# Lucaskabela/UNAST

Hardware: AMD Instinct MI355X
Metric: mel-frames/sec/node (train step, gen+disc) at B=32,T_mel=800; 1/2/4/8-GPU scaling (higher is better)
Workload: dtype bf16x3

## Files before the change

include/unast_hip.h:

```cpp
#ifndef UNAST_HIP_H
#define UNAST_HIP_H
#include <stdint.h>
#ifdef __cplusplus
extern "C" {
#endif

typedef struct ihipStream_t* hipStream_t;

const char* unast_last_error(void);
int unast_version(void);
const char* unast_arch(void);

int unast_gemm(int a_mode, int b_mode, int nsplit,
               const float* A, int lda, const float* B, int ldb, float* C, int ldc,
               int M, int N, int K, int kb_valid,
               int conv_T, int conv_ca, int conv_cb, int conv_shift,
               const float* bias, const float* R, int ldr, const float* G, int ldg, float gate_scale,
               float alpha, int beta, int act,
               float drop_p, unsigned int seed, unsigned int stream_id,
               int splitk, float* splitk_ws, int64_t splitk_ws_floats, float* rowsum_a, int tile_wn, int b_presplit,
               int out_split, double* colstats, hipStream_t stream);

int unast_attn_fwd(int nsplit, const float* Q, int ldq, const float* K, int ldk, const float* V, int ldv, float* O, int ldo,
                   float* LSE, const int* lens_k, int B, int H, int Tq, int Tk, int head_dim, int causal, float scale,
// ... 74 lines not shown
                       hipStream_t stream);

int unast_scalar_combine(const float* a, const float* b, const float* c, float div, float* out, hipStream_t stream);
int unast_masked_mse(const float* gold, const float* pred, const float* mask, int64_t n, double* ws3, float* out, hipStream_t stream);
int unast_speech_loss_fwd(const float* gold, const float* head, int ldh, const float* post, const int* lens, int B, int T, int M,
                          float eos_weight, double* ws, float* loss, hipStream_t stream);
int unast_speech_loss_bwd(const float* gold, const float* head, int ldh, const float* post, const int* lens, int B, int T, int M,
                          float eos_weight, const float* gscale, float* d_head, float* d_post, hipStream_t stream);
int unast_text_loss_fwd(const float* logits, int ldl, const int64_t* gold, int rows, int V, float eos_weight,
                        double* ws, float* loss, hipStream_t stream);
int unast_text_loss_bwd(const float* logits, int ldl, const int64_t* gold, int rows, int V, float eos_weight, const double* ws,
                        const float* gscale, float* dlogits, hipStream_t stream);
int unast_text_head_loss(const float* X, int ldx, const float* W, const float* bias, const int64_t* gold, int rows, int K, int V,
                         float eos_weight, float gscale, float* logits, float* dlogits, int ldl, double* ws, float* loss, hipStream_t stream);
int unast_speech_head_loss(const float* X, int ldx, const float* W, const float* bias, const float* gold, const int* lens, int B, int T, int K, int M,
                           float eos_weight, float gscale, float* head, float* d_head, int ldh, double* ws, hipStream_t stream);
int unast_speech_post_loss(const float* gold, const float* post, const int* lens, int B, int T, int M, float gscale, float* d_post, double* ws,
                           float* loss, hipStream_t stream);
int unast_disc_targets(const int64_t* perm, int n, int B, int flip, float smoothing, float* out, hipStream_t stream);
int unast_randperm(int64_t* out, int n, unsigned int seed, unsigned int stream_id, hipStream_t stream);
int unast_bce_logits(const float* logits, int ldx, const float* targets, int n, const float* gscale, float* loss, float* dlogits,
                     int ldd, hipStream_t stream);

int unast_lstm_fwd(const float* xproj, const float* whh, const float* b_ih, const float* b_hh, const int* lens, float* y, float* gates,
                   float* cs, float* hprev, float* hfinal, int Bd, int T, int ndir, int hidden, int64_t whh_dir_stride,
                   int64_t bias_dir_stride, hipStream_t stream);
int unast_lstm_bwd(const float* dy, const float* dhfinal, const float* whh, const float* gates, const float* cs, const int* lens,
                   float* dgates, int Bd, int T, int ndir, int hidden, int64_t whh_dir_stride, hipStream_t stream);
int unast_leaky_dropout(const float* x, const float* dy, float* out, int rows, int D, float slope, float drop_p, unsigned int seed,
                        unsigned int stream_id, hipStream_t stream);

int unast_conv_fwd(int nsplit, const float* X, int ldx, const float* Wp, float* Y, int ldy, int B, int T, int Cin, int Cout,
                   int taps, int pad_left, const float* bias, int act, const float* R, int ldr, hipStream_t stream);
int unast_maxpool_prev(const float* in, int ld_in, float* out, int ld_out, int B, int T, int C, hipStream_t stream);
int unast_highway_combine(const float* ht, int ld_ht, const float* x, int ld_x, float* out, int ld_out, int rows, int C, hipStream_t stream);
int unast_gru_fwd(const float* xproj, const float* whh, const float* b_hn, float* y, int B, int T, int hidden, hipStream_t stream);

int unast_gru_fwd_train(const float* xproj, const float* whh, const float* b_hn, float* y, float* saved, int B, int T, int hidden,
                        hipStream_t stream);
int unast_gru_bwd(const float* dy, const float* y, const float* saved, const float* whh, float* dx_gates, float* dhn, int B, int T,
                  int hidden, hipStream_t stream);
int unast_maxpool_prev_bwd(const float* dy, int ld_dy, const float* x, int ld_x, float* dx, int ld_dx, int B, int T, int C,
                           int accumulate, int relu_gate, hipStream_t stream);
int unast_relu_bwd(float* dy, int ld_dy, const float* y, int ld_y, int rows, int C, hipStream_t stream);
int unast_highway_combine_bwd(const float* dout, int ld_do, const float* ht, int ld_ht, const float* x, int ld_x, float* dpre, int ld_dp,
                              float* dx, int ld_dx, int rows, int C, hipStream_t stream);
int unast_sum_loss(const float* pred, int ld_pred, const float* mag, int ld_mag, float* dpred, int ld_dpred, int rows, int F, int l2,
                   double* loss, hipStream_t stream);
int unast_split_parts(const float* x, float* hi, float* rest, float* resid, int64_t n, hipStream_t stream);
int unast_conv_dgrad(int nsplit, const float* dY, int lddy, const float* Wp, float* dX, int lddx, int B, int T, int Cin, int Cout,
                     int taps, int pad_left, int beta, hipStream_t stream);
int unast_conv_wgrad(int nsplit, const float* dY, int lddy, const float* X, int ldx, float* dWp, int B, int T, int Cin, int Cout,
                     int taps, int pad_left, float* db, int splitk, float* ws, int64_t ws_floats, hipStream_t stream);

int unast_set_rng_epoch(const unsigned int* counter);

typedef struct {
    const float* A; int lda;
    const float* B; int ldb;
    float* C; int ldc;
    float* rowsum_a;
    int M, N, K;
} unast_wgrad_item;
int unast_wgrad_group(int nsplit, int count, const unast_wgrad_item* items, float* ws, int64_t ws_floats, int target_blocks,
                      hipStream_t stream);
int64_t unast_wgrad_group_ws_floats(int count, const unast_wgrad_item* items, int target_blocks);

int unast_sumsq(const float* g, int64_t n, double* out, hipStream_t stream);
int unast_adamw(float* p, float* g, float* m, float* v, int64_t n, const double* sumsq, float max_norm, float lr,
                float beta1, float beta2, float eps, float weight_decay, int step, float* split_out, int decoupled,
                const float* dev_hyper, int zero_grad, hipStream_t stream);
int unast_split_f32(const float* src, float* dst, int64_t n, hipStream_t stream);
int unast_transpose_split(const float* src_base, float* dst_base, const int* tiles_dev, int ntiles, hipStream_t stream);

int unast_panel_gemm(const float* A, int lda, const void* w_planes, int64_t plane_bytes, float* C, int ldc, int M, int N, int K,
                     const float* bias, const float* R, int ldr, const float* G, int ldg, float gate_scale, int act,
                     float drop_p, unsigned int seed, unsigned int stream_id, int out_split,
                     const float* ln_gamma, const float* ln_beta, float* Y, int ldy, float* mean, float* rstd, float eps,
                     void* gate_bits, int rows_per_wg, hipStream_t stream);
int unast_retile_weights(const float* src_base, void* dst_base, const void* descs_dev, int ndesc, hipStream_t stream);
int unast_panel_gemm_lnbwd(const float* A, int lda, const void* w_planes, int64_t plane_bytes, int M, int K, const float* R, int ldr,
                           const float* z, int ldz, const float* mean, const float* rstd, const float* gamma,
                           float* dz, int lddz, float* dz_drop, int lddrop, float* part, int64_t part_floats,
                           float drop_p, unsigned int seed, unsigned int stream_id, hipStream_t stream);
int64_t unast_panel_gemm_lnbwd_ws_floats(int M);
int unast_layernorm_partials_finalize(const float* part, int nblk, int C, float* dgamma, float* dbeta, hipStream_t stream);
int unast_set_words(unsigned int* dst, const unsigned int* host_words, int n, hipStream_t stream);

int64_t unast_graph_plan_create(void* graph, int nstreams);
int unast_graph_plan_info(int64_t plan, int* out4);
int unast_graph_plan_replay(int64_t plan, hipStream_t origin);
int unast_graph_plan_destroy(int64_t plan);
int unast_graph_plan_allreduces(int64_t plan);
int unast_graph_plan_set_comm(int64_t plan, int64_t comm);
int unast_graph_plan_allreduce_counts(int64_t plan, long long* out, int n);
int unast_capture_reset(void);
int unast_capture_note(hipStream_t stream);
int unast_capture_get_deps(hipStream_t stream, void** out, int cap);
int unast_capture_prune(hipStream_t stream, hipStream_t origin, void** keep, int nkeep);
int unast_graph_plan_streams(int64_t plan);

int unast_comm_unique_id(void* out128);
int64_t unast_comm_init(const void* unique_id128, int rank, int world);
int unast_allreduce(int64_t comm, float* buf, int64_t count, hipStream_t stream);
int unast_allreduce_marker(float* buf, int64_t count, hipStream_t stream);
int unast_comm_destroy(int64_t comm);
// ... 6 lines not shown
```

unast_amd/_lib.py:

```python
import ctypes
import os
import re

_HERE = os.path.dirname(os.path.abspath(__file__))
LIB_PATH = os.environ.get("UNAST_HIP_LIB") or os.path.join(_HERE, "libunast_hip.so")
HEADER_PATH = os.path.join(os.path.dirname(_HERE), "include", "unast_hip.h")

_lib = None
_protos = None


class UnastHipError(RuntimeError):
    pass


def _ctype(decl):
    d = decl.strip()
    if "*" in d or "hipStream_t" in d:
        return ctypes.c_void_p
    base = re.sub(r"\b\w+$", "", d).strip() if len(d.split()) > 1 else d
    base = base.replace("const", "").strip()
    table = {"int": ctypes.c_int, "unsigned int": ctypes.c_uint, "uint32_t": ctypes.c_uint, "float": ctypes.c_float,
             "double": ctypes.c_double, "int64_t": ctypes.c_longlong, "long long": ctypes.c_longlong,
             "uint64_t": ctypes.c_ulonglong, "size_t": ctypes.c_size_t}
    if base not in table:
        raise ValueError("unast_hip.h: cannot map parameter %r" % decl)
    return table[base]


def parse_header(path=HEADER_PATH):
    global _protos
    if _protos is not None:
        return _protos
    src = open(path).read()
    src = re.sub(r"/\*.*?\*/", "", src, flags=re.S)
    src = re.sub(r"//[^\n]*", "", src)
    protos = {}
    for m in re.finditer(r"(const\s+char\s*\*|int64_t|int|void)\s+(unast_\w+)\s*\(([^;{]*?)\)\s*;", src, flags=re.S):
        ret, name, args = m.group(1), m.group(2), m.group(3).strip()
        restype = ctypes.c_char_p if "char" in ret else (None if ret == "void" else (ctypes.c_longlong if ret == "int64_t" else ctypes.c_int))
        argtypes = [] if args in ("", "void") else [_ctype(a) for a in args.split(",")]
        protos[name] = (restype, argtypes)
    _protos = protos
    return protos


def lib():
    return ctypes_lib()


def ctypes_lib():
    global _lib
    if _lib is not None:
        return _lib
    if not os.path.exists(LIB_PATH):
        raise UnastHipError("libunast_hip.so not found at %s — build it with `make -C unast_amd/csrc` "
                            "(or python -c 'import __graft_entry__ as g; g.build()'). There is no fallback path." % LIB_PATH)
    try:
        import torch
        if torch.cuda.is_available():
            torch.cuda.init()
    except ImportError:
        pass
    L = ctypes.CDLL(LIB_PATH)
    for name, (restype, argtypes) in parse_header().items():
        try:
            fn = getattr(L, name)
        except AttributeError:
            raise UnastHipError("libunast_hip.so does not export %s declared in include/unast_hip.h" % name)
        fn.restype = restype
        fn.argtypes = argtypes
    _lib = L
    return L


CAPTURE_NOTE = None


def check(status, what=""):
    if status != 0:
        raise UnastHipError("%s failed (%d): %s" % (what or "unast call", status, lib().unast_last_error().decode()))
    if CAPTURE_NOTE is not None:
        CAPTURE_NOTE()
```

unast_amd/csrc/gemm.hip:

```cpp
#include "common.h"
#include "../../include/unast_hip.h"

#define GBM 128
#define GBK 32
__host__ __device__ constexpr int rc_stride(int rows) { return rows + 16; }
__host__ __device__ constexpr int kc_bytes(int rows) { return rows * GBK * 2; }
__host__ __device__ constexpr int rc_bytes(int rows) { return GBK * rc_stride(rows) * 2; }

enum { OP_KC = 0, OP_KC_CONV = 1, OP_RC = 2, OP_RC_CONV_DGRAD = 3, OP_RC_CONV_WGRAD = 4 };

struct GemmParams {
    const float* A; const float* B; float* C;
    int M, N, K;
    int lda, ldb, ldc;
    int T, ca, cb, shift, KS;
    const float* bias; const float* R; int ldr; const float* G; int ldg; float gate_scale;
    float alpha; int beta; int act;
    uint32_t drop_thresh; float drop_scale; uint32_t seed, stream;
    int kchunk; int atomic; int tiles_m, tiles_n, nsplitk;
    float* slab; int ld_slab; size_t slab_stride;
    int kb_valid;
    float* rowsum_a;
    int group;
    int out_split;
    double* colstats;
};

__device__ __forceinline__ int swz_h(int row) { return (0x1320 >> (((row >> 2) & 3) << 2)) & 3; }
__device__ __forceinline__ int kc_off(int row, int k) {
    return row * 64 + ((((k >> 3) ^ swz_h(row))) << 4) + ((k & 7) << 1);
}

template <int MODE>
__device__ __forceinline__ float4 load_kc(const GemmParams& p, const float* __restrict__ src, int ld, int nrows,
                                          int row, int k, int kend, int conv_rb, int conv_rt) {
    bool ok = row < nrows && k < kend;
    const int rr = min(row, nrows - 1);
    const int kk = min(k, p.K - 4);
    const float* ptr;
    if (MODE == OP_KC) {
        ptr = src + (size_t)rr * ld + kk;
    } else {
        const int j = kk / p.ca;
        const int c = kk - j * p.ca;
        const int ts = conv_rt + j - p.shift;
        ok = ok && ts >= 0 && ts < p.T;
        const int tc = min(max(ts, 0), p.T - 1);
        ptr = src + (size_t)(conv_rb + tc) * ld + c;
    }
    float4 v = *reinterpret_cast<const float4*>(ptr);
    if (!ok) v = make_float4(0.f, 0.f, 0.f, 0.f);
    return v;
// ... 97 lines not shown
    for (int i = 0; i < MI; ++i) {
        const int m = m0 + wm * (16 * MI) + i * 16 + l15;
        if (m >= p.M) continue;
        uint32_t rkey = 0;
        if (p.drop_thresh) rkey = rng_row_key(p.seed, p.stream, (uint32_t)m);
#pragma unroll
        for (int j = 0; j < 4; ++j) {
            const int n = n0 + wn * 64 + j * 16 + 4 * g;
            if (n >= p.N) continue;
            const bool full = (n + 3 < p.N);
            float v[4] = {acc[i][j][0], acc[i][j][1], acc[i][j][2], acc[i][j][3]};
            float gv[4] = {1.f, 1.f, 1.f, 1.f}, rv[4] = {0.f, 0.f, 0.f, 0.f};
            if (p.G) {
                if (vec_g && full) { float4 t4 = *reinterpret_cast<const float4*>(p.G + (size_t)m * p.ldg + n); gv[0] = t4.x; gv[1] = t4.y; gv[2] = t4.z; gv[3] = t4.w; }
                else { for (int r = 0; r < 4; ++r) if (n + r < p.N) gv[r] = p.G[(size_t)m * p.ldg + n + r]; }
            }
            if (p.R && first_split) {
                if (vec_r && full) { float4 t4 = *reinterpret_cast<const float4*>(p.R + (size_t)m * p.ldr + n); rv[0] = t4.x; rv[1] = t4.y; rv[2] = t4.z; rv[3] = t4.w; }
                else { for (int r = 0; r < 4; ++r) if (n + r < p.N) rv[r] = p.R[(size_t)m * p.ldr + n + r]; }
            }
#pragma unroll
            for (int r = 0; r < 4; ++r) {
                float x = v[r] * p.alpha + bias_v[j][r];
                if (p.act == 1) x = fmaxf(x, 0.f);
                if (p.drop_thresh) x = rng_keep(rkey, (uint32_t)(n + r), p.drop_thresh) ? x * p.drop_scale : 0.f;
                if (p.G) x = (gv[r] > 0.f) ? x * p.gate_scale : 0.f;
                v[r] = x + rv[r];
            }
            float* cp = p.C + (size_t)m * p.ldc + n;
            if (p.atomic) {
#pragma unroll
                for (int r = 0; r < 4; ++r)
                    if (n + r < p.N) atomicAdd(cp + r, v[r]);
            } else if (vec_c && full) {
                float4 o = make_float4(v[0], v[1], v[2], v[3]);
                if (p.beta) {
                    float4 c = *reinterpret_cast<const float4*>(cp);
                    o.x += c.x; o.y += c.y; o.z += c.z; o.w += c.w;
                }
                if (p.out_split) *reinterpret_cast<uint4*>(cp) = split_chunk(o);
                else *reinterpret_cast<float4*>(cp) = o;
            } else {
#pragma unroll
                for (int r = 0; r < 4; ++r)
                    if (n + r < p.N) cp[r] = p.beta ? cp[r] + v[r] : v[r];
            }
        }
    }
}

template <int AM, int BMODE, int NSPLIT, int WN, int WM, int FLAGS>
__device__ __forceinline__ void gemm_body(const GemmParams& p, const int pid) {
    constexpr bool FULL = (FLAGS & 1) != 0, BSPLIT = (FLAGS & 2) != 0;
    static_assert(!FULL || ((AM == OP_KC || AM == OP_RC) && (BMODE == OP_KC || BMODE == OP_RC)), "FULL: plain operands only");
    constexpr bool A_KC = (AM == OP_KC || AM == OP_KC_CONV);
    constexpr bool B_KC = (BMODE == OP_KC);
    constexpr int PARTS = (NSPLIT == 3) ? 2 : 1;
    constexpr int NT = 64 * WM * WN;
    constexpr int MI = 8 / WM;
    constexpr int GBN = 64 * WN;
    constexpr int A_BYTES = A_KC ? kc_bytes(GBM) : rc_bytes(GBM);
    constexpr int B_BYTES = B_KC ? kc_bytes(GBN) : rc_bytes(GBN);
    constexpr int A_RCS = rc_stride(GBM), B_RCS = rc_stride(GBN);
    constexpr int A_PASS = (GBM * 8) / NT, B_PASS = (GBN * 8) / NT;
    constexpr int KC_RPP = NT / 8;
    constexpr int A_TPK = GBM / 4, B_TPK = GBN / 4;
    constexpr int A_KPP = NT / A_TPK, B_KPP = NT / B_TPK;
    constexpr int STAGE = (A_BYTES + B_BYTES) * PARTS;
    __shared__ __attribute__((aligned(16))) unsigned char smem[2 * STAGE];

    int tile_m, tile_n, zsplit = 0;
    if (p.tiles_m >= 8 && p.nsplitk == 1 && !p.group) {
        const int G = 8 * p.tiles_n;
        const int grp = pid / G, rem = pid - grp * G;
        tile_m = grp * 8 + (rem & 7);
        tile_n = rem >> 3;
    } else {
        const int ntile = p.tiles_m * p.tiles_n;
        const int g8 = pid & 7, sidx = pid >> 3;
        zsplit = (sidx / ntile) * 8 + g8;
        const int tile = sidx % ntile;
        tile_m = tile % p.tiles_m;
        tile_n = tile / p.tiles_m;
        if (zsplit >= p.nsplitk) return;
    }
    if (tile_m >= p.tiles_m) return;
    const int m0 = tile_m * GBM, n0 = tile_n * GBN;
    const int kbeg = zsplit * p.kchunk;
    const int kend = min(p.K, kbeg + p.kchunk);
    const int nk = (kend - kbeg + GBK - 1) / GBK;

    const int t = threadIdx.x;
    const int lane = t & 63, wave = t >> 6;
    const int wm = wave / WN, wn = wave % WN;
    const int l15 = lane & 15, g = lane >> 4;

    int a_rb[A_PASS], a_rt[A_PASS];
#pragma unroll
    for (int i = 0; i < A_PASS; ++i) { a_rb[i] = 0; a_rt[i] = 0; }
    if (AM == OP_KC_CONV) {
#pragma unroll
        for (int i = 0; i < A_PASS; ++i) {
            int row = min(m0 + (t >> 3) + KC_RPP * i, p.M - 1);
            int b = row / p.T;
            a_rb[i] = b * p.T;
            a_rt[i] = row - b * p.T;
        }
    }
    int b_cj = 0, b_cc = 0;
    if (BMODE == OP_RC_CONV_WGRAD) {
        int row = min(n0 + (t % B_TPK) * 4, p.N - 4);
        b_cj = row / p.cb;
        b_cc = row - b_cj * p.cb;
    }

    uint32_t a_off[A_PASS], b_off[B_PASS];
#pragma unroll
    for (int i = 0; i < A_PASS; ++i)
        a_off[i] = FULL ? 4u * (A_KC ? (uint32_t)(m0 + (t >> 3) + KC_RPP * i) * (uint32_t)p.lda + (t & 7) * 4
                                     : (uint32_t)(t / A_TPK + A_KPP * i) * (uint32_t)p.lda + m0 + (t % A_TPK) * 4) : 0u;
#pragma unroll
    for (int i = 0; i < B_PASS; ++i)
        b_off[i] = FULL ? 4u * (B_KC ? (uint32_t)(n0 + (t >> 3) + KC_RPP * i) * (uint32_t)p.ldb + (t & 7) * 4
                                     : (uint32_t)(t / B_TPK + B_KPP * i) * (uint32_t)p.ldb + n0 + (t % B_TPK) * 4) : 0u;

    auto load_tiles = [&](int kt, float4 (&ra)[A_PASS], float4 (&rb)[B_PASS]) {
        if (FULL) {
            const size_t k0 = (size_t)(kbeg + min(kt, nk - 1) * GBK);
            const char* Ab = reinterpret_cast<const char*>(p.A + (A_KC ? k0 : k0 * (size_t)p.lda));
            const char* Bb = reinterpret_cast<const char*>(p.B + (B_KC ? k0 : k0 * (size_t)p.ldb));
#pragma unroll
            for (int i = 0; i < A_PASS; ++i) ra[i] = *reinterpret_cast<const float4*>(Ab + a_off[i]);
#pragma unroll
            for (int i = 0; i < B_PASS; ++i) rb[i] = *reinterpret_cast<const float4*>(Bb + b_off[i]);
            return;
        }
        const int k0 = kbeg + kt * GBK;
#pragma unroll
        for (int i = 0; i < A_PASS; ++i) {
            if (A_KC) ra[i] = load_kc<AM>(p, p.A, p.lda, p.M, m0 + (t >> 3) + KC_RPP * i, k0 + (t & 7) * 4, kend, a_rb[i], a_rt[i]);
            else      ra[i] = load_rc<AM>(p, p.A, p.lda, p.M, m0 + (t % A_TPK) * 4, k0 + t / A_TPK + A_KPP * i, kend, p.K, 0, 0);
        }
#pragma unroll
        for (int i = 0; i < B_PASS; ++i) {
            if (B_KC) rb[i] = load_kc<BMODE>(p, p.B, p.ldb, p.N, n0 + (t >> 3) + KC_RPP * i, k0 + (t & 7) * 4, kend, 0, 0);
            else      rb[i] = load_rc<BMODE>(p, p.B, p.ldb, p.N, n0 + (t % B_TPK) * 4, k0 + t / B_TPK + B_KPP * i, kend, p.kb_valid, b_cj, b_cc);
        }
    };
    float bsum[4] = {0.f, 0.f, 0.f, 0.f};
    const bool do_rowsum = (AM == OP_RC) && p.rowsum_a && tile_n == 0;
    auto store_tiles = [&](const float4 (&ra)[A_PASS], const float4 (&rb)[B_PASS], unsigned char* sA, unsigned char* sB, bool live) {
#pragma unroll
        for (int i = 0; i < A_PASS; ++i) {
            u32x2 hi, lo;
            if (AM == OP_RC && do_rowsum && live) { bsum[0] += ra[i].x; bsum[1] += ra[i].y; bsum[2] += ra[i].z; bsum[3] += ra[i].w; }
            split4<NSPLIT>(ra[i], hi, lo);
            const int off = A_KC ? kc_off((t >> 3) + KC_RPP * i, (t & 7) * 4) : ((t / A_TPK + A_KPP * i) * A_RCS + (t % A_TPK) * 4) * 2;
            *reinterpret_cast<u32x2*>(sA + off) = hi;
            if (PARTS == 2) *reinterpret_cast<u32x2*>(sA + A_BYTES + off) = lo;
        }
#pragma unroll
        for (int i = 0; i < B_PASS; ++i) {
            u32x2 hi, lo;
            if (BSPLIT) {
                hi[0] = __float_as_uint(rb[i].x); hi[1] = __float_as_uint(rb[i].y);
                lo[0] = __float_as_uint(rb[i].z); lo[1] = __float_as_uint(rb[i].w);
            } else {
                split4<NSPLIT>(rb[i], hi, lo);
            }
            const int off = B_KC ? kc_off((t >> 3) + KC_RPP * i, (t & 7) * 4) : ((t / B_TPK + B_KPP * i) * B_RCS + (t % B_TPK) * 4) * 2;
            *reinterpret_cast<u32x2*>(sB + off) = hi;
            if (PARTS == 2) *reinterpret_cast<u32x2*>(sB + B_BYTES + off) = lo;
        }
    };
    auto frag = [&](const unsigned char* img, bool kc, int rcs, int rbase) -> bf16x8_t {
        if (kc) {
            int row = rbase + l15;
            return *reinterpret_cast<const bf16x8_t*>(img + row * 64 + ((g ^ swz_h(row)) << 4));
        } else {
// ... 150 lines not shown
    const int e = threadIdx.x & 63, zg = threadIdx.x >> 6;
    for (size_t i0 = (size_t)blockIdx.x * 64; i0 < total; i0 += (size_t)gridDim.x * 64) {
        const size_t i = i0 + e;
        float4 a = make_float4(0.f, 0.f, 0.f, 0.f);
        int m = 0, n = 0;
        if (i < total) {
            m = (int)(i / nq); n = (int)(i - (size_t)m * nq) * 4;
            const float* sp = slab + (size_t)m * ld_slab + n;
            int z = zg;
            for (; z + 28 < nsplit; z += 32) {
                float4 v[8];
#pragma unroll
                for (int u = 0; u < 8; ++u) v[u] = *reinterpret_cast<const float4*>(sp + (size_t)(z + 4 * u) * slab_stride);
#pragma unroll
                for (int u = 0; u < 8; ++u) { a.x += v[u].x; a.y += v[u].y; a.z += v[u].z; a.w += v[u].w; }
            }
            for (; z < nsplit; z += 4) {
                const float4 v = *reinterpret_cast<const float4*>(sp + (size_t)z * slab_stride);
                a.x += v.x; a.y += v.y; a.z += v.z; a.w += v.w;
            }
        }
        part[zg][e] = a;
        __syncthreads();
        if (zg == 0 && i < total) {
            const float4 b1 = part[1][e], b2 = part[2][e], b3 = part[3][e];
            const float av[4] = {(a.x + b1.x) + (b2.x + b3.x), (a.y + b1.y) + (b2.y + b3.y), (a.z + b1.z) + (b2.z + b3.z), (a.w + b1.w) + (b2.w + b3.w)};
            float* cp = C + (size_t)m * ldc + n;
#pragma unroll
            for (int r = 0; r < 4; ++r)
                if (n + r < N) cp[r] = beta ? cp[r] + av[r] : av[r];
        }
        __syncthreads();
    }
}

template <int AM, int BMODE, int FLAGS>
static void launch_tile(const GemmParams& p, int nsplit, int wn, dim3 grid, hipStream_t s) {
    if (wn == 4) {
        if (nsplit == 3) hipLaunchKernelGGL((gemm_kernel<AM, BMODE, 3, 4, 2, FLAGS>), grid, dim3(512), 0, s, p);
        else             hipLaunchKernelGGL((gemm_kernel<AM, BMODE, 1, 4, 2, FLAGS>), grid, dim3(512), 0, s, p);
    } else if (wn == 1) {
        if (nsplit == 3) hipLaunchKernelGGL((gemm_kernel<AM, BMODE, 3, 1, 4, FLAGS>), grid, dim3(256), 0, s, p);
        else             hipLaunchKernelGGL((gemm_kernel<AM, BMODE, 1, 1, 4, FLAGS>), grid, dim3(256), 0, s, p);
    } else if (wn == 8) {
        if (nsplit == 3) hipLaunchKernelGGL((gemm_kernel<AM, BMODE, 3, 2, 4, FLAGS>), grid, dim3(512), 0, s, p);
        else             hipLaunchKernelGGL((gemm_kernel<AM, BMODE, 1, 2, 4, FLAGS>), grid, dim3(512), 0, s, p);
    } else {
        if (nsplit == 3) hipLaunchKernelGGL((gemm_kernel<AM, BMODE, 3, 2, 2, FLAGS>), grid, dim3(256), 0, s, p);
        else             hipLaunchKernelGGL((gemm_kernel<AM, BMODE, 1, 2, 2, FLAGS>), grid, dim3(256), 0, s, p);
    }
}
template <int AM, int BMODE, bool WEIGHT_B, bool PLAIN>
static void launch_split(const GemmParams& p, int nsplit, int wn, int flags, dim3 grid, hipStream_t s) {
    const bool fast_tile = (AM == OP_RC) ? (wn == 2) : (wn == 8 || wn == 1);
    if constexpr (PLAIN) {
        if (fast_tile && (flags & 1)) {
            if constexpr (WEIGHT_B) { if (flags & 2) { launch_tile<AM, BMODE, 3>(p, nsplit, wn, grid, s); return; } }
            launch_tile<AM, BMODE, 1>(p, nsplit, wn, grid, s);
            return;
        }
    }
    if constexpr (WEIGHT_B) { if (flags & 2) { launch_tile<AM, BMODE, 2>(p, nsplit, wn, grid, s); return; } }
    launch_tile<AM, BMODE, 0>(p, nsplit, wn, grid, s);
}

static bool aligned16(const void* p) { return (((uintptr_t)p) & 15) == 0; }

static int gemm_run(int a_mode, int b_mode, int nsplit,
                    const float* A, int lda, const float* B, int ldb, float* C, int ldc,
                    int M, int N, int K, int kb_valid,
                    int conv_T, int conv_ca, int conv_cb, int conv_shift, int conv_ks,
                    const float* bias, const float* R, int ldr, const float* G, int ldg, float gate_scale,
                    float alpha, int beta, int act,
                    float drop_p, unsigned int seed, unsigned int stream_id,
                    int splitk, float* splitk_ws, int64_t splitk_ws_floats, float* rowsum_a, int tile_wn, int b_presplit,
                    int out_split, double* colstats, hipStream_t stream) {
    UNAST_REQUIRE(A && B && C, "unast_gemm: null operand");
    UNAST_REQUIRE(!b_presplit || (a_mode == OP_KC || a_mode == OP_KC_CONV), "unast_gemm: a pre-split B is a weight (forward / dgrad forms only)");
    UNAST_REQUIRE(M > 0 && N > 0 && K > 0, "unast_gemm: bad dims M=%d N=%d K=%d", M, N, K);
    UNAST_REQUIRE(nsplit == 1 || nsplit == 3, "unast_gemm: nsplit must be 1 or 3");
    UNAST_REQUIRE(aligned16(A) && aligned16(B) && aligned16(C), "unast_gemm: operands must be 16-byte aligned");
    UNAST_REQUIRE((lda & 3) == 0 && (ldb & 3) == 0, "unast_gemm: lda/ldb must be multiples of 4 (got %d, %d)", lda, ldb);
    UNAST_REQUIRE(splitk >= 1, "unast_gemm: splitk >= 1");
    const bool a_kc = (a_mode == OP_KC || a_mode == OP_KC_CONV), b_kc = (b_mode == OP_KC);
    UNAST_REQUIRE(!(a_kc || b_kc) || ((K & 3) == 0 && K >= 4), "unast_gemm: K-contiguous operands need K %% 4 == 0 (zero-pad the operand; K=%d)", K);
    UNAST_REQUIRE(a_kc || lda >= ((M + 3) & ~3), "unast_gemm: row-contiguous A needs lda >= ceil4(M)");
    UNAST_REQUIRE(b_kc || b_mode != OP_RC || ldb >= ((N + 3) & ~3), "unast_gemm: row-contiguous B needs ldb >= ceil4(N)");
    if (kb_valid <= 0 || kb_valid > K) kb_valid = K;
    UNAST_REQUIRE(!(splitk > 1 && (act || drop_p > 0.f || G || bias || R)),
                  "unast_gemm: split-K supports only the plain alpha/beta epilogue");
    UNAST_REQUIRE(!(splitk > 1 && !splitk_ws && beta == 0), "unast_gemm: atomic split-K (no workspace) accumulates into C: needs beta=1");
    GemmParams p;
    p.A = A; p.B = B; p.C = C; p.M = M; p.N = N; p.K = K; p.lda = lda; p.ldb = ldb; p.ldc = ldc;
    p.T = conv_T > 0 ? conv_T : 1; p.ca = conv_ca > 0 ? conv_ca : 1; p.cb = conv_cb > 0 ? conv_cb : 1;
    p.shift = conv_shift; p.KS = conv_ks;
    p.bias = bias; p.R = R; p.ldr = ldr; p.G = G; p.ldg = ldg; p.gate_scale = gate_scale;
    p.alpha = alpha; p.beta = beta; p.act = act;
    p.drop_thresh = drop_threshold(drop_p); p.drop_scale = drop_p > 0.f ? 1.f / (1.f - drop_p) : 1.f;
    p.seed = seed; p.stream = stream_id; p.group = 0; p.out_split = out_split; p.colstats = colstats;
    UNAST_REQUIRE(!colstats || (a_mode == OP_KC_CONV && b_mode == OP_KC && splitk == 1 && !act && drop_p <= 0.f && !R && !G && beta == 0),
                  "unast_gemm: colstats is for the plain conv forward (bias only)");
    UNAST_REQUIRE(!out_split || ((N & 3) == 0 && (ldc & 3) == 0 && beta == 0 && splitk == 1), "unast_gemm: out_split needs N %% 4 == 0, ldc %% 4 == 0, beta = 0, no split-K");
    int wn = tile_wn;
    if (wn != 1 && wn != 2 && wn != 4 && wn != 8) {
        wn = (a_mode == OP_RC) ? 2 : 8;
        if (a_mode == OP_KC && splitk == 1 && (M + GBM - 1) / GBM * ((N + 127) / 128) <= 128 && N >= 128) wn = 1;
    }
    const int gbn = (wn == 4) ? 256 : (wn == 1) ? 64 : 128;
    p.tiles_m = (M + GBM - 1) / GBM; p.tiles_n = (N + gbn - 1) / gbn;
    int ksteps = (K + GBK - 1) / GBK;
    if (splitk > ksteps) splitk = ksteps;
    int steps_per = (ksteps + splitk - 1) / splitk;
    p.kchunk = steps_per * GBK;
    splitk = (ksteps + steps_per - 1) / steps_per;
    p.slab = nullptr; p.ld_slab = 0; p.slab_stride = 0;
    p.rowsum_a = rowsum_a;
    p.kb_valid = kb_valid;
    UNAST_REQUIRE(!rowsum_a || a_mode == OP_RC, "unast_gemm: rowsum_a needs a row-contiguous A operand (weight-gradient form)");
    p.atomic = 0;
    if (splitk > 1) {
        if (splitk_ws) {
            p.ld_slab = (N + 3) & ~3;
            p.slab_stride = (size_t)M * p.ld_slab;
            UNAST_REQUIRE((int64_t)(p.slab_stride * splitk) <= splitk_ws_floats && ((((uintptr_t)splitk_ws) & 15) == 0),
                          "unast_gemm: split-K workspace too small (need %lld floats) or misaligned", (long long)(p.slab_stride * splitk));
            p.slab = splitk_ws;
        } else {
            p.atomic = 1;
        }
    }
    if (a_mode == OP_KC_CONV) UNAST_REQUIRE((conv_ca & 3) == 0 && K == conv_ks * conv_ca && M % p.T == 0, "unast_gemm: bad conv A geometry");
    if (b_mode == OP_RC_CONV_DGRAD) UNAST_REQUIRE(K == conv_ks * conv_cb, "unast_gemm: bad conv dgrad geometry");
    if (b_mode == OP_RC_CONV_WGRAD) UNAST_REQUIRE((conv_cb & 3) == 0 && N == conv_ks * conv_cb && K % p.T == 0, "unast_gemm: bad conv wgrad geometry");
    p.nsplitk = splitk;
    int flags = b_presplit ? 2 : 0;
    {
        const bool plain = (a_mode == OP_KC || a_mode == OP_RC) && (b_mode == OP_KC || b_mode == OP_RC);
        const uint64_t a_span = a_kc ? (uint64_t)M * lda * 4 : (uint64_t)(GBK + 1) * lda * 4 + (uint64_t)M * 4;
        const uint64_t b_span = b_kc ? (uint64_t)N * ldb * 4 : (uint64_t)(GBK + 1) * ldb * 4 + (uint64_t)N * 4;
        if (plain && M % GBM == 0 && N % gbn == 0 && K % GBK == 0 && kb_valid == K && a_span < (1ull << 32) && b_span < (1ull << 32))
            flags |= 1;
    }
    dim3 grid((p.tiles_m >= 8 && splitk == 1) ? ((p.tiles_m + 7) / 8) * 8 * p.tiles_n : ((splitk + 7) / 8) * 8 * p.tiles_m * p.tiles_n, 1, 1);
    if (a_mode == OP_KC && b_mode == OP_KC) launch_split<OP_KC, OP_KC, true, true>(p, nsplit, wn, flags, grid, stream);
    else if (a_mode == OP_KC && b_mode == OP_RC) launch_split<OP_KC, OP_RC, true, true>(p, nsplit, wn, flags, grid, stream);
    else if (a_mode == OP_RC && b_mode == OP_RC) launch_split<OP_RC, OP_RC, false, true>(p, nsplit, wn, flags, grid, stream);
    else if (a_mode == OP_KC_CONV && b_mode == OP_KC) launch_split<OP_KC_CONV, OP_KC, true, false>(p, nsplit, wn, flags, grid, stream);
    else if (a_mode == OP_KC_CONV && b_mode == OP_RC_CONV_DGRAD) launch_split<OP_KC_CONV, OP_RC_CONV_DGRAD, true, false>(p, nsplit, wn, flags, grid, stream);
    else if (a_mode == OP_RC && b_mode == OP_RC_CONV_WGRAD) launch_split<OP_RC, OP_RC_CONV_WGRAD, false, false>(p, nsplit, wn, flags, grid, stream);
    else return unast_set_error(UNAST_ERR_ARG, "unast_gemm: unsupported operand mode pair (%d,%d)", a_mode, b_mode);
    if (p.slab) {
        size_t work = (size_t)M * (p.ld_slab / 4);
        size_t blocks = (work + 63) / 64;
        if (blocks > 2048) blocks = 2048;
        hipLaunchKernelGGL(splitk_reduce_kernel, dim3((unsigned)blocks), dim3(256), 0, stream, p.slab, p.slab_stride, p.ld_slab, splitk, C, ldc, M, N, beta);
    }
    return unast_check_launch("unast_gemm");
}

extern "C" int unast_gemm(int a_mode, int b_mode, int nsplit,
                          const float* A, int lda, const float* B, int ldb, float* C, int ldc,
                          int M, int N, int K, int kb_valid,
                          int conv_T, int conv_ca, int conv_cb, int conv_shift,
                          const float* bias, const float* R, int ldr, const float* G, int ldg, float gate_scale,
                          float alpha, int beta, int act,
                          float drop_p, unsigned int seed, unsigned int stream_id,
                          int splitk, float* splitk_ws, int64_t splitk_ws_floats, float* rowsum_a, int tile_wn, int b_presplit,
                          int out_split, double* colstats, hipStream_t stream) {
    return gemm_run(a_mode, b_mode, nsplit, A, lda, B, ldb, C, ldc, M, N, K, kb_valid, conv_T, conv_ca, conv_cb, conv_shift, 5,
                    bias, R, ldr, G, ldg, gate_scale, alpha, beta, act, drop_p, seed, stream_id, splitk, splitk_ws, splitk_ws_floats,
                    rowsum_a, tile_wn, b_presplit, out_split, colstats, stream);
}

extern "C" int unast_conv_fwd(int nsplit, const float* X, int ldx, const float* Wp, float* Y, int ldy, int B, int T, int Cin, int Cout,
                              int taps, int pad_left, const float* bias, int act, const float* R, int ldr, hipStream_t stream) {
    UNAST_REQUIRE(taps >= 1 && taps <= 16, "unast_conv_fwd: 1..16 taps (got %d)", taps);
    UNAST_REQUIRE(B > 0 && T > 0 && Cin > 0 && Cout > 0 && (Cin & 3) == 0, "unast_conv_fwd: bad dims B=%d T=%d Cin=%d Cout=%d (Cin %% 4 == 0)", B, T, Cin, Cout);
    UNAST_REQUIRE(pad_left >= 0 && pad_left < taps, "unast_conv_fwd: pad_left must be in [0, taps)");
    UNAST_REQUIRE(ldx >= Cin && ldy >= Cout && (!R || ldr >= Cout), "unast_conv_fwd: row strides shorter than the rows");
    UNAST_REQUIRE((long long)B * T <= 0x7FFFFFFF && (long long)taps * Cin <= 0x7FFFFFFF, "unast_conv_fwd: problem too large");
    return gemm_run(OP_KC_CONV, OP_KC, nsplit, X, ldx, Wp, taps * Cin, Y, ldy, B * T, Cout, taps * Cin, 0, T, Cin, 0, pad_left, taps,
                    bias, R, ldr, nullptr, 0, 1.f, 1.f, 0, act, 0.f, 0u, 0u, 1, nullptr, 0, nullptr, 0, 0, 0, nullptr, stream);
}

extern "C" int unast_conv_dgrad(int nsplit, const float* dY, int lddy, const float* Wp, float* dX, int lddx, int B, int T, int Cin, int Cout,
                                int taps, int pad_left, int beta, hipStream_t stream) {
    UNAST_REQUIRE(taps >= 1 && taps <= 16, "unast_conv_dgrad: 1..16 taps (got %d)", taps);
    UNAST_REQUIRE(B > 0 && T > 0 && Cin > 0 && Cout > 0 && (Cin & 3) == 0 && (Cout & 3) == 0,
                  "unast_conv_dgrad: bad dims B=%d T=%d Cin=%d Cout=%d (both %% 4 == 0)", B, T, Cin, Cout);
    UNAST_REQUIRE(pad_left >= 0 && pad_left < taps, "unast_conv_dgrad: pad_left must be in [0, taps)");
    UNAST_REQUIRE(lddy >= Cout && lddx >= Cin && (beta == 0 || beta == 1), "unast_conv_dgrad: row strides shorter than the rows, or beta not 0 / 1");
    UNAST_REQUIRE((long long)B * T <= 0x7FFFFFFF && (long long)taps * Cout <= 0x7FFFFFFF, "unast_conv_dgrad: problem too large");
    return gemm_run(OP_KC_CONV, OP_RC_CONV_DGRAD, nsplit, dY, lddy, Wp, 4, dX, lddx, B * T, Cin, taps * Cout, 0, T, Cout, Cout, taps - 1 - pad_left, taps,
                    nullptr, nullptr, 0, nullptr, 0, 1.f, 1.f, beta, 0, 0.f, 0u, 0u, 1, nullptr, 0, nullptr, 0, 0, 0, nullptr, stream);
// ... 90 lines not shown
```

unast_amd/ops.py:

```python
import os as _os

import torch

from . import config
from ._lib import lib, check

OP_KC, OP_KC_CONV, OP_RC, OP_RC_CONV_DGRAD, OP_RC_CONV_WGRAD = 0, 1, 2, 3, 4


def _p(t):
    return None if t is None else t.data_ptr()


_raw_stream = getattr(torch._C, "_cuda_getCurrentRawStream", None)


def _stream():
    if _raw_stream is not None:
        return _raw_stream(torch.cuda.current_device())
    return torch.cuda.current_stream().cuda_stream


_F32 = torch.float32
_LN_WS = {}
# ... 344 lines not shown
def panel_gemm(A, wplanes, C, N, bias=None, R=None, G=None, gate_scale=1.0, act=0, drop_p=0.0, seed=0, stream_id=0, out_split=False,
               ln=None, rows_per_wg=0, K=None, gate_bits=None):
    M = A.shape[0]
    K = A.shape[1] if K is None else K
    g = b = Y = mean = rstd = None
    eps, ldy = 0.0, 0
    if ln is not None:
        g, b, Y, mean, rstd, eps = ln
        ldy = Y.stride(0)
    PANEL_LAUNCHES[0 if K <= 256 else 1] += 1
    if _PANEL_TRACE:
        print("panel_gemm M=%d N=%d K=%d lda=%d ldc=%d bias=%s R=%s G=%s act=%d drop=%.2f split=%d ln=%s bits=%s rows=%d" % (
            M, N, K, A.stride(0), C.stride(0), bias is not None, R is not None, G is not None, act, drop_p, out_split, ln is not None,
            None if gate_bits is None else gate_bits.numel(), rows_per_wg), flush=True)
    check(lib().unast_panel_gemm(_p(A), A.stride(0), wplanes[0], wplanes[1], _p(C), C.stride(0), M, N, K, _p(bias), _p(R),
                                 R.stride(0) if R is not None else 0, _p(G), G.stride(0) if G is not None else 0, gate_scale, act,
                                 drop_p, seed & 0xFFFFFFFF, stream_id, int(out_split), _p(g), _p(b), _p(Y), ldy, _p(mean), _p(rstd), eps,
                                 _p(gate_bits), rows_per_wg, _stream()), "unast_panel_gemm")
    if _PANEL_TRACE:
        torch.cuda.synchronize()
    return C


def conv_fwd(x3d, Wp, bias, out, pad_left, colstats=None):
    B, T, Cin = x3d.shape
    Cout = Wp.shape[0]
    gemm(OP_KC_CONV, OP_KC, x3d, x3d.stride(1), Wp, 5 * Cin, out, out.stride(1), B * T, Cout, 5 * Cin,
         conv=(T, Cin, 0, pad_left), bias=bias, colstats=colstats)
    return out


def conv_dgrad(dy3d, Wp, dx, pad_left, beta=0):
    B, T, Cout = dy3d.shape
    Cin = Wp.shape[2]
    gemm(OP_KC_CONV, OP_RC_CONV_DGRAD, dy3d, dy3d.stride(1), Wp, 4, dx, dx.stride(1), B * T, Cin, 5 * Cout,
         conv=(T, Cout, Cout, 4 - pad_left), beta=beta)
    return dx


def conv_wgrad(dy3d, x3d, dWp, pad_left, db=None):
    B, T, Cout = dy3d.shape
    Cin = x3d.shape[2]
    sk = _splitk_for(Cout, 5 * Cin, B * T)
    if db is not None and deterministic_sums() and dy3d.is_contiguous():
        def both():
            gemm(OP_RC, OP_RC_CONV_WGRAD, dy3d, dy3d.stride(1), x3d, x3d.stride(1), dWp, 5 * Cin, Cout, 5 * Cin, B * T,
                 conv=(T, 0, Cin, pad_left), beta=1, splitk=sk)
            colsum(dy3d.view(B * T, Cout), db)
        _on_wgrad_stream(both, B * T, dWp.data_ptr(), dy3d, x3d)
        return dWp
    _on_wgrad_stream(lambda: gemm(OP_RC, OP_RC_CONV_WGRAD, dy3d, dy3d.stride(1), x3d, x3d.stride(1), dWp, 5 * Cin, Cout, 5 * Cin, B * T,
                                  conv=(T, 0, Cin, pad_left), beta=1, splitk=sk, rowsum_a=db), B * T, dWp.data_ptr(), dy3d, x3d)
    return dWp


def attn_fwd(Q, K, V, O, LSE, lens_k, B, H, Tq, Tk, causal, drop_p=0.0, seed=0, stream_id=0, nsplit=None, qkv_split=False):
    check(lib().unast_attn_fwd(nsplit or config.NSPLIT, _p(Q), Q.stride(0), _p(K), K.stride(0), _p(V), V.stride(0), _p(O), O.stride(0),
                               _p(LSE), _p(lens_k), B, H, Tq, Tk, 64, int(causal), 0.125, drop_p, seed & 0xFFFFFFFF, stream_id,
                               int(qkv_split), _stream()), "unast_attn_fwd")


def attn_bwd(Q, K, V, O, dO, LSE, delta_ws, dQ, dK, dV, lens_k, B, H, Tq, Tk, causal, drop_p=0.0, seed=0, stream_id=0, nsplit=None, qkv_split=False, lens_q=None):
    fused = config.ATTN_FUSED_BWD and not deterministic_sums()
    check(lib().unast_attn_bwd(nsplit or config.NSPLIT, _p(Q), Q.stride(0), _p(K), K.stride(0), _p(V), V.stride(0), _p(O), O.stride(0),
                               _p(dO), dO.stride(0), _p(LSE), _p(delta_ws), _p(dQ), dQ.stride(0), _p(dK), dK.stride(0), _p(dV),
                               dV.stride(0), _p(lens_k), B, H, Tq, Tk, 64, int(causal), 0.125, drop_p, seed & 0xFFFFFFFF, stream_id,
                               (2 if config.ATTN_BWD_TERMS == 2 else 1) if fused else 0, int(qkv_split),
                               _p(lens_q) if fused else None, _stream()), "unast_attn_bwd")


def layernorm_fwd(z, gamma, beta, y, mean, rstd, eps=1e-5):
    rows, C = z.shape
    check(lib().unast_layernorm_fwd(_p(z), _p(gamma), _p(beta), _p(y), _p(mean), _p(rstd), rows, C, eps, _stream()), "unast_layernorm_fwd")


def layernorm_bwd(dy, z, gamma, mean, rstd, dz, dz_drop=None, dgamma=None, dbeta=None, drop_p=0.0, seed=0, stream_id=0):
    rows, C = z.shape
    ws, ws_n = None, 0
    if dgamma is not None:
        ws_n = _LN_WS.get((rows, C))
        if ws_n is None:
            ws_n = _LN_WS[(rows, C)] = lib().unast_layernorm_bwd_ws_floats(rows, C)
        ws = torch.empty(ws_n, dtype=torch.float32, device=z.device)
    check(lib().unast_layernorm_bwd(_p(dy), _p(z), _p(gamma), _p(mean), _p(rstd), _p(dz), _p(dz_drop), _p(dgamma), _p(dbeta), _p(ws), ws_n,
                                    rows, C, drop_p, seed & 0xFFFFFFFF, stream_id, 0 if dgamma is not None else 1, _stream()), "unast_layernorm_bwd")
    if dgamma is not None:
        _on_wgrad_stream(lambda: check(lib().unast_layernorm_bwd_finalize(_p(ws), ws_n, rows, C, _p(dgamma), _p(dbeta), _stream()),
                                       "unast_layernorm_bwd_finalize"), rows, dgamma.data_ptr(), ws)


def colsum(x2d, out):
    rows, C = x2d.shape
    if deterministic_sums():
        ws_n = lib().unast_colsum_det_ws_floats(rows, C)
        ws = torch.empty(ws_n, dtype=torch.float32, device=x2d.device)
        check(lib().unast_colsum_det(_p(x2d), x2d.stride(0), rows, C, _p(out), _p(ws), ws_n, _stream()), "unast_colsum_det")
        return
    check(lib().unast_colsum_f32(_p(x2d), x2d.stride(0), rows, C, _p(out), _stream()), "unast_colsum_f32")


def bn_fwd(x2d, gamma, beta, y, mean, rstd, running_mean, running_var, ws, act, drop_p=0.0, seed=0, stream_id=0, eps=1e-5, momentum=0.1, have_sums=False,
           num_batches_tracked=None):
    rows, C = x2d.shape
    check(lib().unast_bn_fwd(_p(x2d), _p(gamma), _p(beta), _p(y), _p(mean), _p(rstd), _p(running_mean), _p(running_var), _p(ws), rows, C,
                             eps, momentum, act, drop_p, seed & 0xFFFFFFFF, stream_id, int(have_sums), _p(num_batches_tracked), _stream()), "unast_bn_fwd")

# ... 495 lines not shown
```

Before: 946,700.

## Add fast full-tile path for conv GEMM forms using buffer-load gathers

```diff
diff --git a/include/unast_hip.h b/include/unast_hip.h
--- a/include/unast_hip.h
+++ b/include/unast_hip.h
@@ -150,6 +150,7 @@
                      int taps, int pad_left, int beta, hipStream_t stream);
 int unast_conv_wgrad(int nsplit, const float* dY, int lddy, const float* X, int ldx, float* dWp, int B, int T, int Cin, int Cout,
                      int taps, int pad_left, float* db, int splitk, float* ws, int64_t ws_floats, hipStream_t stream);
+long long unast_conv_fast_launches(int form);
 
 int unast_set_rng_epoch(const unsigned int* counter);
 
diff --git a/unast_amd/_lib.py b/unast_amd/_lib.py
--- a/unast_amd/_lib.py
+++ b/unast_amd/_lib.py
@@ -36,9 +36,9 @@
     src = re.sub(r"/\*.*?\*/", "", src, flags=re.S)
     src = re.sub(r"//[^\n]*", "", src)
     protos = {}
-    for m in re.finditer(r"(const\s+char\s*\*|int64_t|int|void)\s+(unast_\w+)\s*\(([^;{]*?)\)\s*;", src, flags=re.S):
+    for m in re.finditer(r"(const\s+char\s*\*|int64_t|long\s+long|int|void)\s+(unast_\w+)\s*\(([^;{]*?)\)\s*;", src, flags=re.S):
         ret, name, args = m.group(1), m.group(2), m.group(3).strip()
-        restype = ctypes.c_char_p if "char" in ret else (None if ret == "void" else (ctypes.c_longlong if ret == "int64_t" else ctypes.c_int))
+        restype = ctypes.c_char_p if "char" in ret else (None if ret == "void" else (ctypes.c_longlong if ret == "int64_t" or ret.startswith("long") else ctypes.c_int))
         argtypes = [] if args in ("", "void") else [_ctype(a) for a in args.split(",")]
         protos[name] = (restype, argtypes)
     _protos = protos
diff --git a/unast_amd/csrc/gemm.hip b/unast_amd/csrc/gemm.hip
--- a/unast_amd/csrc/gemm.hip
+++ b/unast_amd/csrc/gemm.hip
@@ -1,3 +1,4 @@
+#include <atomic>
 #include "common.h"
 #include "../../include/unast_hip.h"
 
@@ -201,7 +202,10 @@
 template <int AM, int BMODE, int NSPLIT, int WN, int WM, int FLAGS>
 __device__ __forceinline__ void gemm_body(const GemmParams& p, const int pid) {
     constexpr bool FULL = (FLAGS & 1) != 0, BSPLIT = (FLAGS & 2) != 0;
-    static_assert(!FULL || ((AM == OP_KC || AM == OP_RC) && (BMODE == OP_KC || BMODE == OP_RC)), "FULL: plain operands only");
+    static_assert(!FULL || ((AM == OP_KC || AM == OP_RC) && (BMODE == OP_KC || BMODE == OP_RC)) || (AM == OP_KC_CONV && BMODE == OP_KC) ||
+                  (AM == OP_KC_CONV && BMODE == OP_RC_CONV_DGRAD) || (AM == OP_RC && BMODE == OP_RC_CONV_WGRAD), "FULL: plain operands or one of the three conv forms");
+    constexpr bool CONV_A = FULL && AM == OP_KC_CONV, DGRAD_B = FULL && BMODE == OP_RC_CONV_DGRAD, WGRAD_B = FULL && BMODE == OP_RC_CONV_WGRAD;
+    constexpr uint32_t GATHER_OOB = 0x80000000u;
     constexpr bool A_KC = (AM == OP_KC || AM == OP_KC_CONV);
     constexpr bool B_KC = (BMODE == OP_KC);
     constexpr int PARTS = (NSPLIT == 3) ? 2 : 1;
@@ -269,11 +273,74 @@
         a_off[i] = FULL ? 4u * (A_KC ? (uint32_t)(m0 + (t >> 3) + KC_RPP * i) * (uint32_t)p.lda + (t & 7) * 4
                                      : (uint32_t)(t / A_TPK + A_KPP * i) * (uint32_t)p.lda + m0 + (t % A_TPK) * 4) : 0u;
 #pragma unroll
-    for (int i = 0; i < B_PASS; ++i)
-        b_off[i] = FULL ? 4u * (B_KC ? (uint32_t)(n0 + (t >> 3) + KC_RPP * i) * (uint32_t)p.ldb + (t & 7) * 4
-                                     : (uint32_t)(t / B_TPK + B_KPP * i) * (uint32_t)p.ldb + n0 + (t % B_TPK) * 4) : 0u;
+    for (int i = 0; i < B_PASS; ++i) {
+        if (CONV_A && B_KC)  b_off[i] = 4u * ((uint32_t)min(n0 + (t >> 3) + KC_RPP * i, p.N - 1) * (uint32_t)p.ldb + (t & 7) * 4);
+        else if (DGRAD_B)    b_off[i] = 4u * ((uint32_t)(t / B_TPK + B_KPP * i) * (uint32_t)(p.KS * p.N) + ((n0 + (t % B_TPK) * 4 < p.N) ? n0 + (t % B_TPK) * 4 : 0));
+        else if (WGRAD_B)    b_off[i] = 4u * (uint32_t)((t / B_TPK + B_KPP * i + b_cj - p.shift) * p.ldb + b_cc);
+        else b_off[i] = FULL ? 4u * (B_KC ? (uint32_t)(n0 + (t >> 3) + KC_RPP * i) * (uint32_t)p.ldb + (t & 7) * 4
+                                          : (uint32_t)(t / B_TPK + B_KPP * i) * (uint32_t)p.ldb + n0 + (t % B_TPK) * 4) : 0u;
+    }
+    int kl = 0, c_j = 0, c_c0 = 0;
+    uint32_t a_mask[A_PASS], a_vo[A_PASS];
+    int b_ts[B_PASS];
+    __amdgpu_buffer_rsrc_t g_rs;
+    if constexpr (CONV_A) {
+        g_rs = __builtin_amdgcn_make_buffer_rsrc(const_cast<float*>(p.A), 0, (int)(((size_t)(p.M - 1) * p.lda + p.ca) * 4), 0x00020000);
+#pragma unroll
+        for (int i = 0; i < A_PASS; ++i) {
+            uint32_t m = 0;
+            for (int j = 0; j < p.KS; ++j) {
+                const int ts = a_rt[i] + j - p.shift;
+                if (ts >= 0 && ts < p.T) m |= 1u << j;
+            }
+            a_mask[i] = m; a_vo[i] = GATHER_OOB;
+        }
+    }
+    if constexpr (WGRAD_B) {
+        g_rs = __builtin_amdgcn_make_buffer_rsrc(const_cast<float*>(p.B), 0, (int)(((size_t)(p.K - 1) * p.ldb + p.cb) * 4), 0x00020000);
+        const int tbeg = kbeg % p.T;
+#pragma unroll
+        for (int i = 0; i < B_PASS; ++i) {
+            int tt = tbeg + t / B_TPK + B_KPP * i;
+            if (tt >= p.T) tt -= p.T;
+            b_ts[i] = tt + b_cj - p.shift;
+        }
+    }
 
     auto load_tiles = [&](int kt, float4 (&ra)[A_PASS], float4 (&rb)[B_PASS]) {
+        if constexpr (CONV_A) {
+            if (c_c0 == 0) {
+                const uint32_t tap = (uint32_t)(4 * (c_j - p.shift) * p.lda);
+#pragma unroll
+                for (int i = 0; i < A_PASS; ++i) a_vo[i] = ((a_mask[i] >> c_j) & 1u) ? a_off[i] + tap : GATHER_OOB;
+            }
+#pragma unroll
+            for (int i = 0; i < A_PASS; ++i) ra[i] = __builtin_bit_cast(float4, __builtin_amdgcn_raw_buffer_load_b128(g_rs, (int)a_vo[i], 4 * c_c0, 0));
+            const char* Bb = reinterpret_cast<const char*>(B_KC ? p.B + (size_t)kl * GBK : p.B + (size_t)(c_c0 * p.KS + (p.KS - 1 - c_j)) * (size_t)p.N);
+#pragma unroll
+            for (int i = 0; i < B_PASS; ++i) rb[i] = *reinterpret_cast<const float4*>(Bb + b_off[i]);
+            if (kl + 1 < nk) {
+                ++kl; c_c0 += GBK;
+                if (c_c0 == p.ca) { c_c0 = 0; ++c_j; }
+            }
+            return;
+        }
+        if constexpr (WGRAD_B) {
+            const uint32_t k0 = (uint32_t)(kbeg + kl * GBK);
+            const char* Ab = reinterpret_cast<const char*>(p.A + (size_t)k0 * (size_t)p.lda);
+#pragma unroll
+            for (int i = 0; i < A_PASS; ++i) ra[i] = *reinterpret_cast<const float4*>(Ab + a_off[i]);
+            const uint32_t kb = 4u * k0 * (uint32_t)p.ldb;
+#pragma unroll
+            for (int i = 0; i < B_PASS; ++i)
+                rb[i] = __builtin_bit_cast(float4, __builtin_amdgcn_raw_buffer_load_b128(g_rs, (int)(((uint32_t)b_ts[i] < (uint32_t)p.T) ? b_off[i] + kb : GATHER_OOB), 0, 0));
+            if (kl + 1 < nk) {
+                ++kl;
+#pragma unroll
+                for (int i = 0; i < B_PASS; ++i) { b_ts[i] += GBK; if (b_ts[i] >= p.T + b_cj - p.shift) b_ts[i] -= p.T; }
+            }
+            return;
+        }
         if (FULL) {
             const size_t k0 = (size_t)(kbeg + min(kt, nk - 1) * GBK);
             const char* Ab = reinterpret_cast<const char*>(p.A + (A_KC ? k0 : k0 * (size_t)p.lda));
@@ -530,7 +597,21 @@
 }
 template <int AM, int BMODE, bool WEIGHT_B, bool PLAIN>
 static void launch_split(const GemmParams& p, int nsplit, int wn, int flags, dim3 grid, hipStream_t s) {
-    const bool fast_tile = (AM == OP_RC) ? (wn == 2) : (wn == 8 || wn == 1);
+    const bool fast_tile = (AM == OP_RC) ? (wn == 2) : (wn == 8 || (PLAIN && wn == 1));
+    if constexpr (!PLAIN) {
+        if (fast_tile && (flags & 1)) {
+            constexpr int WM = (AM == OP_RC) ? 2 : 4;
+            constexpr int F = 1 | (WEIGHT_B ? 2 : 0);
+            if (WEIGHT_B && (flags & 2)) {
+                if (nsplit == 3) hipLaunchKernelGGL((gemm_kernel<AM, BMODE, 3, 2, WM, F>), grid, dim3(128 * WM), 0, s, p);
+                else             hipLaunchKernelGGL((gemm_kernel<AM, BMODE, 1, 2, WM, F>), grid, dim3(128 * WM), 0, s, p);
+            } else {
+                if (nsplit == 3) hipLaunchKernelGGL((gemm_kernel<AM, BMODE, 3, 2, WM, 1>), grid, dim3(128 * WM), 0, s, p);
+                else             hipLaunchKernelGGL((gemm_kernel<AM, BMODE, 1, 2, WM, 1>), grid, dim3(128 * WM), 0, s, p);
+            }
+            return;
+        }
+    }
     if constexpr (PLAIN) {
         if (fast_tile && (flags & 1)) {
             if constexpr (WEIGHT_B) { if (flags & 2) { launch_tile<AM, BMODE, 3>(p, nsplit, wn, grid, s); return; } }
@@ -543,6 +624,11 @@
 }
 
 static bool aligned16(const void* p) { return (((uintptr_t)p) & 15) == 0; }
+
+static std::atomic<long long> g_conv_fast[3];
+extern "C" long long unast_conv_fast_launches(int form) {
+    return (form >= 0 && form < 3) ? g_conv_fast[form].load(std::memory_order_relaxed) : -1;
+}
 
 static int gemm_run(int a_mode, int b_mode, int nsplit,
                     const float* A, int lda, const float* B, int ldb, float* C, int ldc,
@@ -618,6 +704,16 @@
         const uint64_t b_span = b_kc ? (uint64_t)N * ldb * 4 : (uint64_t)(GBK + 1) * ldb * 4 + (uint64_t)N * 4;
         if (plain && M % GBM == 0 && N % gbn == 0 && K % GBK == 0 && kb_valid == K && a_span < (1ull << 32) && b_span < (1ull << 32))
             flags |= 1;
+        const uint64_t GIB2 = 1ull << 31;
+        int form = -1;
+        if (a_mode == OP_KC_CONV && M % GBM == 0 && conv_ca % GBK == 0 && splitk == 1 && wn == 8 && ((uint64_t)(M - 1) * lda + conv_ca) * 4 < GIB2) {
+            if (b_mode == OP_KC && (uint64_t)N * ldb * 4 < GIB2) form = 0;
+            if (b_mode == OP_RC_CONV_DGRAD && conv_cb == conv_ca && (N & 3) == 0 && (uint64_t)K * N * 4 < GIB2) form = 1;
+        }
+        if (a_mode == OP_RC && b_mode == OP_RC_CONV_WGRAD && M % GBM == 0 && N % 128 == 0 && K % GBK == 0 && kb_valid == K && p.T >= GBK && wn == 2 &&
+            a_span < (1ull << 32) && ((uint64_t)(K - 1) * ldb + conv_cb) * 4 < GIB2)
+            form = 2;
+        if (form >= 0) { flags |= 1; g_conv_fast[form].fetch_add(1, std::memory_order_relaxed); }
     }
     dim3 grid((p.tiles_m >= 8 && splitk == 1) ? ((p.tiles_m + 7) / 8) * 8 * p.tiles_n : ((splitk + 7) / 8) * 8 * p.tiles_m * p.tiles_n, 1, 1);
     if (a_mode == OP_KC && b_mode == OP_KC) launch_split<OP_KC, OP_KC, true, true>(p, nsplit, wn, flags, grid, stream);
diff --git a/unast_amd/ops.py b/unast_amd/ops.py
--- a/unast_amd/ops.py
+++ b/unast_amd/ops.py
@@ -420,6 +420,10 @@
     _on_wgrad_stream(lambda: gemm(OP_RC, OP_RC_CONV_WGRAD, dy3d, dy3d.stride(1), x3d, x3d.stride(1), dWp, 5 * Cin, Cout, 5 * Cin, B * T,
                                   conv=(T, 0, Cin, pad_left), beta=1, splitk=sk, rowsum_a=db), B * T, dWp.data_ptr(), dy3d, x3d)
     return dWp
+
+
+def conv_fast_launches(form):
+    return int(lib().unast_conv_fast_launches(form))
 
 
 def attn_fwd(Q, K, V, O, LSE, lens_k, B, H, Tq, Tk, causal, drop_p=0.0, seed=0, stream_id=0, nsplit=None, qkv_split=False):
```

Result: faster. 956,700 (median of 6 runs) (+1.1%).
